# mehta-lab/dynamorph

Measured on AMD Instinct MI355X. Metric: cell-patches/sec (128x128x2) VQ-VAE fwd+bwd, higher is better.
Workload: dtype f32; 1 GPU; C3: VQ_VAE training step (forward + backward + fused Adam), 2x128x128 fp32 synthetic patches; per_gpu_batch=2048, global_batch=2048, parallelism=dp1, hip_graph=True, fused_trainer=True, backward_products=f32

## Files before the change

### dynamorph_amd/csrc/conv_mfma.hip

```cpp
#include "dm_common.h"
#include "tile.h"
#include "mfma_util.h"

int dm_generic_conv_slabs(int B, int per_tile);
int dm_generic_conv(int form, const Operand &in, const WeightView &wv, float *out, const Epilogue &ep, int B, int Cphys,
                    int CIN, int NOUT, int H, int W, int taps, int nslabs, int per_tile, hipStream_t st);
bool dm_wide_conv_ok(int form, int H, int W);
int dm_wide_conv_slabs(int form, int B, int H, int W, int per_tile);
long long dm_wide_conv_scratch_floats(int form, int CIN, int NOUT, int taps);
int dm_wide_conv(int form, const Operand &in, const WeightView &wv, float *scratch, float *out, const Epilogue &ep, int B,
                 int Cphys, int CIN, int NOUT, int H, int W, int taps, int nslabs, int per_tile, hipStream_t st);

bool dm_conv4x4s2_patch_forward(const Operand &in, const WeightView &wv, float *out, const Epilogue &ep, int B, int Cphys, int CIN,
                                int NOUT, int H, int W, int per_tile, int nslabs, hipStream_t stream, int *rc);

namespace {

enum { SIDE_NONE = 0, SIDE_MASK = 1, SIDE_ALL = 2 };

template <int SIDE> struct EpiIn { f32x4 m; };
template <> struct EpiIn<SIDE_ALL> { f32x4 m, r, q; };

constexpr unsigned DM_RSRC_FLAGS = 0x00020000u;
constexpr int DM_VOFF_NONE = 0x40000000;

__device__ __forceinline__ __amdgpu_buffer_rsrc_t sample_rsrc(const float *base, long long sample_elems, int b)
{
    return base ? __builtin_amdgcn_make_buffer_rsrc(const_cast<float *>(base + sample_elems * b), 0,
                                                    (int)(sample_elems * 4), DM_RSRC_FLAGS)
                : __builtin_amdgcn_make_buffer_rsrc(nullptr, 0, 0, DM_RSRC_FLAGS);
}

template <int SIDE> struct EpiCtx {
    __amdgpu_buffer_rsrc_t out_r, m_r, r_r, q_r;
    __device__ __forceinline__ void rebase(const Epilogue &ep, float *out, long long sample_elems, int b)
    {
        out_r = sample_rsrc(out, sample_elems, b);
        if constexpr (SIDE != SIDE_NONE) m_r = sample_rsrc(ep.mask.p0, sample_elems, b);
        if constexpr (SIDE == SIDE_ALL) {
            r_r = sample_rsrc(ep.resid, sample_elems, b);
            q_r = sample_rsrc(ep.stat_q, sample_elems, b);
        }
    }
};

template <int SIDE>
__device__ __forceinline__ void epilogue_loads(EpiIn<SIDE> &e, const EpiCtx<SIDE> &cx, int voff)
{
    if constexpr (SIDE != SIDE_NONE) e.m = __builtin_amdgcn_raw_buffer_load_b128(cx.m_r, voff, 0, 0);
    if constexpr (SIDE == SIDE_ALL) {
        e.r = __builtin_amdgcn_raw_buffer_load_b128(cx.r_r, voff, 0, 0);
        e.q = __builtin_amdgcn_raw_buffer_load_b128(cx.q_r, voff, 0, 0);
    }
}

__device__ __forceinline__ void mask_coef(const Epilogue &ep, int b, int chan, float &c0, float &c2)
{
    c0 = ep.mask.p0 ? 1.f : 0.f; c2 = ep.mask.p0 ? 0.f : 1.f;
    if (ep.mask.p0 && ep.mask.mode >= DM_LOAD_AFFINE) {
        const float *cf = ep.mask.coef + (long long)b * ep.mask.coef_bstride + chan * 4;
        c0 = cf[0]; c2 = cf[2];
    }
}

template <int SIDE>
__device__ __forceinline__ void epilogue_tail(f32x4 v, const Epilogue &ep, const EpiCtx<SIDE> &cx, const EpiIn<SIDE> &e,
                                              float mc0, float mc2, int voff, double &s1, double &s2)
{
    f32x4 q = v;
    if constexpr (SIDE != SIDE_NONE) {
        const f32x4 mv = mc0 * e.m + mc2;
        v.x = mv.x > 0.f ? v.x : 0.f; v.y = mv.y > 0.f ? v.y : 0.f;
        v.z = mv.z > 0.f ? v.z : 0.f; v.w = mv.w > 0.f ? v.w : 0.f;
    }
    if constexpr (SIDE == SIDE_ALL) v += e.r;
    __builtin_amdgcn_raw_buffer_store_b128(v, cx.out_r, voff, 0, 0);
    if (ep.stats) {
        q = v;
        if constexpr (SIDE == SIDE_MASK) { if (ep.stat_q) q = e.m; }
        if constexpr (SIDE == SIDE_ALL) { if (ep.stat_q) q = e.q; }
        s1 += (double)((v.x + v.y) + (v.z + v.w));
        s2 += (double)((v.x * q.x + v.y * q.y) + (v.z * q.z + v.w * q.w));
    }
}

__device__ __forceinline__ f32x4 bias_relu(f32x4 v, const Epilogue &ep, float bias)
{
    v += bias;
    if (ep.relu) v = dm_relu4(v);
    return v;
}

template <int NTT, bool PIX>
__device__ __forceinline__ void stats_reduce(double (&s1)[NTT], double (&s2)[NTT], double (*s_stat)[2],
                                             const Epilogue &ep, int NCH, long long slab)
{
    const int lane = threadIdx.x & 63, wave = threadIdx.x >> 6;
#pragma unroll
    for (int t = 0; t < NTT; ++t) {
        double a = dm_row_sum_f64(s1[t]), c = dm_row_sum_f64(s2[t]);
        if (PIX) {
            a += __shfl_xor(a, 1, 64); c += __shfl_xor(c, 1, 64);
            a += __shfl_xor(a, 2, 64); c += __shfl_xor(c, 2, 64);
        }
        if (lane < 16) {
            s_stat[(wave * NTT + t) * 16 + lane][0] = a;
            s_stat[(wave * NTT + t) * 16 + lane][1] = c;
        }
    }
    __syncthreads();
    for (int ch = threadIdx.x; ch < NCH; ch += DM_BLOCK) {
        const int n = PIX ? ch * 4 : ch;
        const int t = n >> 4, l = n & 15;
        double a = 0.0, c = 0.0;
#pragma unroll
        for (int w = 0; w < 4; ++w) {
            a += s_stat[(w * NTT + t) * 16 + l][0];
            c += s_stat[(w * NTT + t) * 16 + l][1];
        }
        ep.stats[(slab * NCH + ch) * 2 + 0] = a;
        ep.stats[(slab * NCH + ch) * 2 + 1] = c;
    }
}

__device__ __forceinline__ void zero_unowned_slabs(const Epilogue &ep, int NCH, int nslabs)
{
    for (int t2 = blockIdx.x + gridDim.x; t2 < nslabs; t2 += gridDim.x)
        for (int i = threadIdx.x; i < NCH * 2; i += DM_BLOCK) ep.stats[(long long)t2 * NCH * 2 + i] = 0.0;
}

template <int CIN, int NT, int TH, int TW, int SIDE, int WPS, bool BB>
__global__ __launch_bounds__(DM_BLOCK, WPS)
void conv4x4s2_kernel(Operand in, WeightView wv, float *__restrict__ out, Epilogue ep, int Cphys, int NOUT, int H,
                      int W, int ntiles, int nslabs, int per_tile)
{
    constexpr int IH = 2 * TH + 2, RS = 2 * TW + 8, COLS4 = RS / 4, PS = IH * RS;
    constexpr int KS = CIN * 4, CG = TW / 16, MT = TH * CG, MTW = MT / 4;
    constexpr int MP = NT == 1 ? 2 : 1;
    static_assert(MTW % MP == 0 && MTW >= MP, "M tiles per wave");
    __shared__ __attribute__((aligned(16))) float tile[CIN * PS];
    __shared__ __attribute__((aligned(16))) float s_coef[DM_COEF_MAX_C * 4];
    __shared__ double s_stat[4 * NT * 16][2];

    const int Ho = H >> 1, Wo = W >> 1;
    const int tiles_x = Wo / TW, tiles_y = Ho / TH;
    const int lane = threadIdx.x & 63, wave = threadIdx.x >> 6, m = lane & 15, kq = lane >> 4;

    TileStage<CIN, IH, COLS4, RS, PS, false> stage;
    stage.init(H, W);
    int tidx = blockIdx.x, b = 0, oy0 = 0, ox0 = 0;
    if (tidx < ntiles) {
        int t = tidx;
        ox0 = (t % tiles_x) * TW; t /= tiles_x;
        oy0 = (t % tiles_y) * TH; b = t / tiles_y;
        stage.issue(in, b, Cphys, H, W, 2 * oy0 - 1, 2 * ox0 - 4);
        stage_coef(s_coef, in, b, Cphys);
    }

    static_assert(!BB || NT == 1, "bias_border: one N tile");
    float tb00 = 0.f, tb01 = 0.f, tb02 = 0.f, tb10 = 0.f, tb11 = 0.f, tb12 = 0.f, tb20 = 0.f, tb21 = 0.f, tb22 = 0.f;
    if constexpr (BB) {
        const float *tp = ep.bias_border + (m < NOUT ? m : 0);
        tb00 = tp[0 * NOUT]; tb01 = tp[1 * NOUT]; tb02 = tp[2 * NOUT];
        tb10 = tp[3 * NOUT]; tb11 = tp[4 * NOUT]; tb12 = tp[5 * NOUT];
        tb20 = tp[6 * NOUT]; tb21 = tp[7 * NOUT]; tb22 = tp[8 * NOUT];
    }
    float wreg[NT][KS], bias[NT], mc0[NT], mc2[NT];
#pragma unroll
    for (int t = 0; t < NT; ++t) {
        const int n = 16 * t + m;
        const int nc = n < NOUT ? n : 0;
        bias[t] = ep.bias ? ep.bias[nc] : 0.f;
        mask_coef(ep, 0, nc, mc0[t], mc2[t]);
#pragma unroll
        for (int s = 0; s < KS; ++s)
            wreg[t][s] = n < NOUT ? wv.w[wv.off + n * wv.sn + (s >> 2) * wv.sc + (s & 3) * wv.sky + kq * wv.skx] : 0.f;
    }

    double s1[NT], s2[NT];
#pragma unroll
    for (int t = 0; t < NT; ++t) { s1[t] = 0.0; s2[t] = 0.0; }
    const int abase = 2 * m + kq + 3;
    auto off = [](int s) { return (s >> 2) * PS + (s & 3) * RS; };
    EpiCtx<SIDE> cx;
    const long long sample_elems = (long long)NOUT * Ho * Wo;
    int chan_off[NT];
#pragma unroll
    for (int t = 0; t < NT; ++t) chan_off[t] = 16 * t + m < NOUT ? ((16 * t + m) * Ho * Wo + 4 * kq) * 4 : DM_VOFF_NONE;
    while (tidx < ntiles) {
        __syncthreads();
        stage.commit(tile, s_coef, Cphys, H, W, 2 * oy0 - 1, 2 * ox0 - 4, in.mode);
        __syncthreads();
        const int cb = b, cy0 = oy0, cx0 = ox0;
        const int next = tidx + gridDim.x;
        {
            int t = next < ntiles ? next : tidx;
            ox0 = (t % tiles_x) * TW; t /= tiles_x;
            oy0 = (t % tiles_y) * TH; b = t / tiles_y;
        }
        const auto scx = stage.begin(in, next < ntiles, b, Cphys, H, W, 2 * oy0 - 1, 2 * ox0 - 4);
        const bool recoef = next < ntiles && coef_changes(in, cb, b);
        f32x4 cfn = {1.f, 0.f, 0.f, 0.f};
        if (recoef) cfn = coef_fetch(in, b, Cphys);
        if (SIDE != SIDE_NONE && ep.mask.p0 && ep.mask.coef_bstride) {
#pragma unroll
            for (int t = 0; t < NT; ++t) mask_coef(ep, cb, 16 * t + m < NOUT ? 16 * t + m : 0, mc0[t], mc2[t]);
        }
        cx.rebase(ep, out, sample_elems, cb);
        constexpr int NP = MTW / MP, NE = decltype(stage)::N;
#pragma unroll
        for (int p = 0; p < NP; ++p) {
#pragma unroll
            for (int e = 0; e < NE; ++e)
                if (e >= p * NE / NP && e < (p + 1) * NE / NP) stage.issue_one(e, scx);
            const float *ap[MP];
            int o[MP][NT];
            EpiIn<SIDE> e[MP][NT];
#pragma unroll
            for (int i = 0; i < MP; ++i) {
                const int ti = wave + 4 * (MP * p + i);
                const int r = ti / CG, cg = ti % CG;
                ap[i] = tile + (2 * r) * RS + 32 * cg + abase;
#pragma unroll
                for (int t = 0; t < NT; ++t) {
                    o[i][t] = chan_off[t] + ((cy0 + r) * Wo + cx0 + 16 * cg) * 4;
                    epilogue_loads<SIDE>(e[i][t], cx, o[i][t]);
                }
            }
            f32x4 acc[MP][NT];
#pragma unroll
            for (int i = 0; i < MP; ++i)
#pragma unroll
                for (int t = 0; t < NT; ++t) acc[i][t] = (f32x4){0.f, 0.f, 0.f, 0.f};
            mfma_tiles<MP, NT, KS, 4>(ap, wreg, acc, off);
#pragma unroll
            for (int i = 0; i < MP; ++i)
#pragma unroll
                for (int t = 0; t < NT; ++t)
                {
                    f32x4 v = acc[i][t];
                    if constexpr (BB) {
                        const int ti = wave + 4 * (MP * p + i);
                        const int y = cy0 + ti / CG, xq = cx0 + 16 * (ti % CG) + 4 * kq;
                        const bool r0 = y == 0, r2 = y == Ho - 1;
                        const float bl = r0 ? tb00 : (r2 ? tb20 : tb10);
                        const float bm = r0 ? tb01 : (r2 ? tb21 : tb11);
                        const float br = r0 ? tb02 : (r2 ? tb22 : tb12);
                        v += (f32x4){xq == 0 ? bl : bm, bm, bm, xq + 3 == Wo - 1 ? br : bm};
                        v = bias_relu(v, ep, 0.f);
                    } else {
                        v = bias_relu(v, ep, bias[t]);
                    }
                    epilogue_tail<SIDE>(v, ep, cx, e[i][t], mc0[t], mc2[t], o[i][t], s1[t], s2[t]);
                }
        }
        if (per_tile && ep.stats) {
            stats_reduce<NT, false>(s1, s2, s_stat, ep, NOUT, tidx);
#pragma unroll
            for (int t = 0; t < NT; ++t) { s1[t] = 0.0; s2[t] = 0.0; }
        }
        if (recoef) coef_put(s_coef, in, cfn, Cphys);
        tidx = next;
    }
    if (ep.stats && !per_tile) {
        stats_reduce<NT, false>(s1, s2, s_stat, ep, NOUT, blockIdx.x);
        zero_unowned_slabs(ep, NOUT, nslabs);
    }
}

template <int CIN, int TH, int WPS>
__global__ __launch_bounds__(DM_BLOCK, WPS)
void conv4x4s2_pair_kernel(Operand in, WeightView wv, float *__restrict__ out, Epilogue ep, int Cphys, int H, int W, int ntiles,
                           int nslabs, int per_tile)
{
    constexpr int NOUT = 8, TW = 64;
    constexpr int IH = 2 * TH + 2, RS = 2 * TW + 8, COLS4 = RS / 4, PS = IH * RS;
    constexpr int KS = CIN * 2, RPW = TH / 4;
    static_assert(TH % 4 == 0, "rows over four waves");
    __shared__ __attribute__((aligned(16))) float tile[CIN * PS + 64];
    __shared__ __attribute__((aligned(16))) float s_coef[DM_COEF_MAX_C * 4];
    __shared__ double s_stat[4 * 16][2];

    const int Ho = H >> 1, Wo = W >> 1;
    const int tiles_x = Wo / TW, tiles_y = Ho / TH;
    const int lane = threadIdx.x & 63, wave = threadIdx.x >> 6, m = lane & 15, kq = lane >> 4;
    const int co = m & 7, mj = m >> 3;
    const int kyl = kq >> 1, col = kq & 1;

    TileStage<CIN, IH, COLS4, RS, PS, false> stage;
    stage.init(H, W);
    int tidx = blockIdx.x, b = 0, oy0 = 0, ox0 = 0;
    if (tidx < ntiles) {
        int t = tidx;
        ox0 = (t % tiles_x) * TW; t /= tiles_x;
        oy0 = (t % tiles_y) * TH; b = t / tiles_y;
        stage.issue(in, b, Cphys, H, W, 2 * oy0 - 1, 2 * ox0 - 4);
        stage_coef(s_coef, in, b, Cphys);
    }
    if (threadIdx.x < 64) tile[CIN * PS + threadIdx.x] = 0.f;

    const float *tp = ep.bias_border + co;
    const float tb00 = tp[0 * NOUT], tb01 = tp[1 * NOUT], tb02 = tp[2 * NOUT];
    const float tb10 = tp[3 * NOUT], tb11 = tp[4 * NOUT], tb12 = tp[5 * NOUT];
    const float tb20 = tp[6 * NOUT], tb21 = tp[7 * NOUT], tb22 = tp[8 * NOUT];
    float wc[1][KS], ws[1][KS];
#pragma unroll
    for (int s = 0; s < KS; ++s) {
        const int c = s >> 1, ky = 2 * (s & 1) + kyl;
        const long long base = wv.off + co * wv.sn + c * wv.sc + ky * wv.sky;
        wc[0][s] = wv.w[base + (col + (mj ? 0 : 2)) * wv.skx];
        ws[0][s] = wv.w[base + (col + (mj ? 2 : 0)) * wv.skx];
    }
    float mc0, mc2;
    mask_coef(ep, 0, co, mc0, mc2);
// ... 615 lines not shown
                        }
                    } else {
#pragma unroll
                        for (int i = 0; i < MP; ++i) v[i] = acc[i][0];
                    }
#pragma unroll
                    for (int i = 0; i < MP; ++i) {
                        const f32x4 pv = lane_xor8(v[i]);
                        epilogue_tail<SIDE_MASK>(pxl ? (f32x4){pv.z, v[i].z, pv.w, v[i].w} : (f32x4){v[i].x, pv.x, v[i].y, pv.y}, ep, cx,
                                                 e[i], mc0, mc2, obase[i] + py * OW * 4, s1, s2);
                    }
                }
            }
            }
            __syncthreads();
            p ^= 1;
            tidx += gridDim.x;
        }
        for (int w = 0; w < RW + 1; ++w) __syncthreads();
        if (ep.stats) {
            double a = s1, c = s2;
            a += __shfl_xor(a, 16, 64); c += __shfl_xor(c, 16, 64);
            a += __shfl_xor(a, 32, 64); c += __shfl_xor(c, 32, 64);
            a += __shfl_xor(a, 8, 64); c += __shfl_xor(c, 8, 64);
            if (lane < CX) { s_stat[rw * 16 + lane][0] = a; s_stat[rw * 16 + lane][1] = c; }
        }
        __syncthreads();
        if (ep.stats && threadIdx.x < CX) {
            double ta = 0.0, tc = 0.0;
#pragma unroll
            for (int w = 0; w < RW; ++w) { ta += s_stat[w * 16 + threadIdx.x][0]; tc += s_stat[w * 16 + threadIdx.x][1]; }
            ep.stats[((long long)blockIdx.x * CX + threadIdx.x) * 2 + 0] = ta;
            ep.stats[((long long)blockIdx.x * CX + threadIdx.x) * 2 + 1] = tc;
        }
    }
    float *slab = wslabs + (long long)blockIdx.x * (CD * N);
    for (int i = threadIdx.x; i < NTT * 256; i += 768) {
        const int j = i & 3, l = (i >> 2) & 63, t = i >> 8;
        slab[(4 * (l >> 4) + j) * N + 16 * t + (l & 15)] = fb_lds[i];
    }
}

struct ConvArgs {
    Operand in; WeightView wv; float *out; Epilogue ep;
    int B, Cphys, CIN, NOUT, H, W, per_tile;
    hipStream_t stream;
};

int side_mode(const Epilogue &ep)
{
    if (!ep.mask.p0 && !ep.resid && !ep.stat_q) return SIDE_NONE;
    if (ep.mask.p0 && !ep.resid && (!ep.stat_q || ep.stat_q == ep.mask.p0)) return SIDE_MASK;
    return SIDE_ALL;
}

int conv_grid(int ntiles, int wgs_per_cu, int per_tile, int npass = 1)
{
    if (per_tile && npass > 1) return ntiles;
    const int cap = 256 * wgs_per_cu;
    return ntiles < cap ? ntiles : cap;
}

int conv_slabs(int ntiles, int per_tile) { return per_tile ? ntiles : (ntiles < 256 * 3 ? ntiles : 256 * 3); }

constexpr int lds_wgs(int lds_bytes) { return (160 * 1024) / (lds_bytes + 3072); }
constexpr int clampi(int v, int lo, int hi) { return v < lo ? lo : (v > hi ? hi : v); }

constexpr int conv_wps(int lds_bytes, int weights, int tile_f4, bool two, int mp, int nt, int side)
{
    const int stage = ((tile_f4 + DM_BLOCK - 1) / DM_BLOCK) * (two ? 9 : 5);
    const int epi = mp * nt * (6 + (side == SIDE_ALL ? 12 : (side == SIDE_MASK ? 4 : 0)));
    const int est = weights + stage + epi + 48;
    return clampi(lds_wgs(lds_bytes), 1, est > 145 ? 2 : 3);
}

int conv4_tw(int CIN, int Wo)
{
    const int cap = CIN <= 5 ? 64 : (CIN <= 8 ? 32 : 16);
    return Wo < cap ? Wo : cap;
}

template <int CIN, int TW>
void launch_conv4(const ConvArgs &a)
{
    constexpr int TH = 8;
    constexpr int F4 = CIN * (2 * TH + 2) * ((2 * TW + 8) / 4), LDS = 16 * F4;
    const int ntiles = a.B * ((a.H / 2) / TH) * ((a.W / 2) / TW);
#define DM_L4(SIDE_)                                                                                              \
    {                                                                                                             \
        constexpr int WPS = conv_wps(LDS, CIN * 4, F4, false, 2, 1, SIDE_);                                       \
                                           \
        if (SIDE_ == SIDE_NONE && CIN <= 4 && TW == 64 && a.NOUT == 8 && a.ep.bias_border && !a.ep.relu)             \
            hipLaunchKernelGGL((conv4x4s2_pair_kernel<CIN <= 4 ? CIN : 1, TH, WPS>),                                   \
                               dim3(conv_grid(ntiles, WPS, a.per_tile)), dim3(DM_BLOCK), 0, a.stream, a.in, a.wv,     \
                               a.out, a.ep, a.Cphys, a.H, a.W, ntiles, conv_slabs(ntiles, a.per_tile), a.per_tile);    \
        else if (SIDE_ == SIDE_NONE && CIN <= 5 && a.ep.bias_border)                                              \
            hipLaunchKernelGGL((conv4x4s2_kernel<CIN, 1, TH, TW, SIDE_NONE, WPS, true>),                              \
                               dim3(conv_grid(ntiles, WPS, a.per_tile)), dim3(DM_BLOCK), 0, a.stream, a.in, a.wv,     \
                               a.out, a.ep, a.Cphys, a.NOUT, a.H, a.W, ntiles, conv_slabs(ntiles, a.per_tile),        \
                               a.per_tile);                                                                           \
        else                                                                                                      \
            hipLaunchKernelGGL((conv4x4s2_kernel<CIN, 1, TH, TW, SIDE_, WPS, false>),                                 \
                               dim3(conv_grid(ntiles, WPS, a.per_tile)), dim3(DM_BLOCK), 0, a.stream, a.in, a.wv,     \
                               a.out, a.ep, a.Cphys, a.NOUT, a.H, a.W, ntiles, conv_slabs(ntiles, a.per_tile),        \
                               a.per_tile);                                                                           \
    }
    switch (side_mode(a.ep)) {
    case SIDE_NONE: DM_L4(SIDE_NONE) break;
    case SIDE_MASK: DM_L4(SIDE_MASK) break;
    default: DM_L4(SIDE_ALL)
    }
#undef DM_L4
}

int conv3_tw(int W, int CIN)
{
    const int cap = CIN >= 32 ? 16 : (CIN >= 16 ? 32 : 64);
    return W < cap ? W : cap;
}
constexpr int conv3_th(int TW, int CIN) { return (TW == 16 && CIN < 32) ? 16 : 8; }

template <int CIN, int NT, int NPASS, int TAPS, bool PIX, int TW>
void launch_conv3(const ConvArgs &a)
{
    constexpr int TH = conv3_th(TW, CIN);
    constexpr int PADR = TAPS == 9 ? 1 : 0;
    constexpr int F4 = CIN * (TH + 2 * PADR) * ((TW + 8 * PADR) / 4), LDS = 16 * F4 + 2048;
    const int ntiles = a.B * (a.H / TH) * (a.W / TW);
    const int side = side_mode(a.ep);
    const bool two = a.in.mode == DM_LOAD_AFFINE2;
#define DM_L3(TWO_, SIDE_)                                                                                        \
    {                                                                                                             \
        constexpr int WPS = conv_wps(LDS, NT * (CIN / 4) * TAPS, F4, TWO_, NT == 1 ? 2 : 1, NT, SIDE_);          \
        hipLaunchKernelGGL((conv3x3_kernel<CIN, NT, NPASS, TAPS, PIX, TH, TW, TWO_, SIDE_, WPS>),                 \
                           dim3(conv_grid(ntiles, WPS, a.per_tile, NPASS)), dim3(DM_BLOCK), 0, a.stream, a.in, a.wv, \
                           a.out, a.ep, a.Cphys, a.NOUT, a.H, a.W, ntiles, conv_slabs(ntiles, a.per_tile), a.per_tile); \
    }
    if (!two && side == SIDE_NONE) DM_L3(false, SIDE_NONE)
    else if (!two && side == SIDE_MASK) DM_L3(false, SIDE_MASK)
    else if (two && side != SIDE_ALL) DM_L3(true, SIDE_MASK)
    else DM_L3(true, SIDE_ALL)
#undef DM_L3
}

template <int CIN, int COUT, int TW>
void launch_convT_phase(const ConvArgs &a)
{
    constexpr int TH = conv3_th(TW, CIN);
    constexpr int F4 = CIN * (TH + 2) * ((TW + 8) / 4), LDS = 16 * F4 + 2048;
    constexpr int KSW = (CIN / 4) * (COUT == 16 ? 4 : 6) * (COUT == 16 ? 4 : 2);
    const int ntiles = a.B * (a.H / TH) * (a.W / TW);
    const int side = side_mode(a.ep);
    const bool two = a.in.mode == DM_LOAD_AFFINE2;
#define DM_LP(TWO_, SIDE_)                                                                                        \
    {                                                                                                             \
        constexpr int WPS = clampi(conv_wps(LDS, KSW, F4, TWO_, 2, COUT == 16 ? 2 : 1, SIDE_), 1, 2);             \
        hipLaunchKernelGGL((convT_phase_kernel<CIN, COUT, TH, TW, TWO_, SIDE_, WPS>),                             \
                           dim3(conv_grid(ntiles, WPS, a.per_tile)), dim3(DM_BLOCK), 0, a.stream, a.in, a.wv,     \
                           a.out, a.ep, a.Cphys, a.H, a.W, ntiles, conv_slabs(ntiles, a.per_tile));               \
    }
    if (!two && side == SIDE_NONE) DM_LP(false, SIDE_NONE)
    else if (!two && side == SIDE_MASK) DM_LP(false, SIDE_MASK)
    else if (two && side != SIDE_ALL) DM_LP(true, SIDE_MASK)
    else DM_LP(true, SIDE_ALL)
#undef DM_LP
}

}

static int conv_common_checks(const char *who, const dm_operand *in, const dm_weight_view *w, float *out,
                              const dm_epilogue *ep, int B, int CIN, int NOUT, int H, int W)
{
    if (dm_check_operand(in, who)) return -1;
    DM_REQUIRE(w && w->w && out, "%s: NULL weight or output", who);
    DM_REQUIRE(B > 0 && CIN > 0 && NOUT > 0 && H > 0 && W > 0, "%s: bad shape", who);
    DM_REQUIRE((long long)B * (CIN > NOUT ? CIN : NOUT) * H * W < (1LL << 31),
               "%s: tensor too large for 32-bit element offsets", who);
    DM_REQUIRE(CIN - (in->ones_channel ? 1 : 0) > 0, "%s: no physical input channel", who);
    DM_REQUIRE((long long)NOUT * H * W * 4 < DM_VOFF_NONE, "%s: one output sample must stay below 1 GiB", who);
    if (ep && ep->mask.p0 && dm_check_operand(&ep->mask, who)) return -1;
    DM_REQUIRE(!(ep && ep->mask.p0 && ep->mask.ones_channel), "%s: mask operand cannot have a ones channel", who);
    DM_REQUIRE(!(ep && ep->mask.p0 && ep->mask.mode != DM_LOAD_IDENT && ep->mask.mode != DM_LOAD_AFFINE),
               "%s: mask operand must be IDENT or AFFINE", who);
    return 0;
}

static int conv4_fast_tw(int CIN, int NOUT, int H, int W)
{
    const int Wo = W / 2, Ho = H / 2;
    const int TW = conv4_tw(CIN, Wo);
    if (H % 16 || W % 32 || NOUT > 16 || (TW != 16 && TW != 32 && TW != 64) || Ho % 8 || Wo % TW) return 0;
    return TW;
}

static bool conv4_has_kernel(int CIN, int TW)
{
    if (CIN >= 1 && CIN <= 5) return TW == 64 || TW == 32 || TW == 16;
    if (CIN == 8) return TW == 32 || TW == 16;
    return CIN == 16 && TW == 16;
}

extern "C" int dm_conv4x4s2_num_blocks(int B, int CIN, int NOUT, int H, int W, int per_tile)
{
    if (B <= 0 || H <= 0 || W <= 0 || (H & 1) || (W & 1)) return -1;
    const int TW = conv4_fast_tw(CIN, NOUT, H, W);
    if (TW && conv4_has_kernel(CIN, TW)) return conv_slabs(B * ((H / 2) / 8) * ((W / 2) / TW), per_tile);
    if (dm_wide_conv_ok(0, H, W)) return dm_wide_conv_slabs(0, B, H, W, per_tile);
    return dm_generic_conv_slabs(B, per_tile);
}

extern "C" int64_t dm_conv4x4s2_scratch_floats(int CIN, int NOUT, int H, int W, int fallback)
{
    if (CIN <= 0 || NOUT <= 0 || !dm_wide_conv_ok(0, H, W)) return 0;
    const int TW = conv4_fast_tw(CIN, NOUT, H, W);
    if (TW && conv4_has_kernel(CIN, TW) && !fallback) return 0;
    return dm_wide_conv_scratch_floats(0, CIN, NOUT, 16);
}

extern "C" int dm_conv4x4s2(const dm_operand *in, const dm_weight_view *w, float *out, const dm_epilogue *ep,
                            int B, int CIN, int NOUT, int H, int W, void *stream)
{
    if (conv_common_checks("dm_conv4x4s2", in, w, out, ep, B, CIN, NOUT, H, W)) return -1;
    DM_REQUIRE(H % 2 == 0 && W % 2 == 0, "dm_conv4x4s2: H and W must be even (got %dx%d)", H, W);
    ConvArgs a{to_dev(in), to_dev(w), out, to_dev(ep), B, CIN - (in->ones_channel ? 1 : 0), CIN, NOUT, H, W,
               ep ? ep->stats_per_tile : 0, (hipStream_t)stream};
    {
        int rc = 0;
        if (dm_conv4x4s2_patch_forward(a.in, a.wv, out, a.ep, B, a.Cphys, CIN, NOUT, H, W, a.per_tile,
                                       dm_conv4x4s2_num_blocks(B, CIN, NOUT, H, W, a.per_tile), a.stream, &rc))
            return rc;
    }
    const int TW = conv4_fast_tw(CIN, NOUT, H, W);
    const bool border_ok = !(ep && ep->bias_border) || (CIN <= 5 && !ep->mask.p0 && !ep->resid && !ep->stat_q && W / 2 >= 8);
    if (TW && conv4_has_kernel(CIN, TW) && in->mode != DM_LOAD_AFFINE2 && border_ok) {
#define DM_C4(C, T) if (CIN == C && TW == T) { launch_conv4<C, T>(a); return dm_launch_status("dm_conv4x4s2"); }
        DM_C4(3, 64) DM_C4(3, 32) DM_C4(3, 16)
        DM_C4(4, 64) DM_C4(4, 32) DM_C4(4, 16)
        DM_C4(5, 64) DM_C4(5, 32) DM_C4(5, 16)
        DM_C4(2, 64) DM_C4(2, 32) DM_C4(2, 16)
        DM_C4(1, 64) DM_C4(1, 32) DM_C4(1, 16)
        DM_C4(8, 32) DM_C4(8, 16)
        DM_C4(16, 16)
#undef DM_C4
    }
    const int nslabs = dm_conv4x4s2_num_blocks(B, CIN, NOUT, H, W, a.per_tile);
    if (dm_wide_conv_ok(0, H, W) && w->scratch && w->scratch_floats >= dm_wide_conv_scratch_floats(0, CIN, NOUT, 16))
        dm_wide_conv(0, a.in, a.wv, w->scratch, out, a.ep, B, a.Cphys, CIN, NOUT, H, W, 16, nslabs, a.per_tile, a.stream);
    else
        dm_generic_conv(0, a.in, a.wv, out, a.ep, B, a.Cphys, CIN, NOUT, H, W, 16, nslabs, a.per_tile, a.stream);
    return dm_launch_status("dm_conv4x4s2");
}

static bool conv3_fast_tileable(int CIN, int H, int W)
{
    const int TW = conv3_tw(W, CIN), TH = conv3_th(TW, CIN);
    return (TW == 16 || TW == 32 || TW == 64) && W % TW == 0 && H % TH == 0 && CIN % 4 == 0 && CIN <= 32;
}

static bool conv3_has_kernel(int CIN, int NOUT, int H, int W, int taps, bool pix, int per_tile)
{
    if (!conv3_fast_tileable(CIN, H, W)) return false;
    const int TW = conv3_tw(W, CIN), NTT = (NOUT + 15) / 16;
    const bool t13 = TW == 16 || TW == 32;
    if (pix && CIN == 16 && (NOUT == 32 || NOUT == 64) && t13 && !per_tile) return true;
    if (!pix && taps == 9) return t13 && ((CIN == 16 && (NTT == 1 || NTT == 2)) || (CIN == 32 && NTT == 1));
    if (!pix && taps == 1) return t13 && ((CIN == 32 && NTT == 1) || (CIN == 16 && NTT == 2));
    if (pix && taps == 9) {
        if (CIN == 16 && NTT == 2) return true;
        if (CIN == 16 && NTT == 4) return t13;
        if (CIN == 8 && NTT == 1) return TW == 32 || TW == 64;
        if (CIN == 4 && NTT == 1) return TW == 64;
    }
    return false;
}

extern "C" int dm_conv3x3_num_blocks(int B, int CIN, int NOUT, int H, int W, int taps, int pixel_shuffle, int per_tile)
{
    if (B <= 0 || H <= 0 || W <= 0) return -1;
    if (conv3_has_kernel(CIN, NOUT, H, W, taps, pixel_shuffle != 0, per_tile)) {
        const int TW = conv3_tw(W, CIN), TH = conv3_th(TW, CIN);
        return conv_slabs(B * (H / TH) * (W / TW), per_tile);
    }
    const int form = pixel_shuffle ? 2 : 1;
    if (dm_wide_conv_ok(form, H, W)) return dm_wide_conv_slabs(form, B, H, W, per_tile);
    return dm_generic_conv_slabs(B, per_tile);
}

extern "C" int64_t dm_conv3x3_scratch_floats(int CIN, int NOUT, int H, int W, int taps, int pixel_shuffle, int per_tile)
{
    const int form = pixel_shuffle ? 2 : 1;
    if (CIN <= 0 || NOUT <= 0 || (taps != 9 && taps != 1) || !dm_wide_conv_ok(form, H, W)) return 0;
    if (conv3_has_kernel(CIN, NOUT, H, W, taps, pixel_shuffle != 0, per_tile)) return 0;
    return dm_wide_conv_scratch_floats(form, CIN, NOUT, taps);
}

extern "C" int dm_conv3x3(const dm_operand *in, const dm_weight_view *w, float *out, const dm_epilogue *ep,
                          int B, int CIN, int NOUT, int H, int W, int taps, int pixel_shuffle, void *stream)
{
    if (conv_common_checks("dm_conv3x3", in, w, out, ep, B, CIN, NOUT, H, W)) return -1;
    DM_REQUIRE(taps == 9 || taps == 1, "dm_conv3x3: taps must be 9 or 1");
    DM_REQUIRE(!pixel_shuffle || (taps == 9 && NOUT % 4 == 0), "dm_conv3x3: pixel_shuffle needs taps=9, NOUT%%4==0");
    DM_REQUIRE(!in->ones_channel, "dm_conv3x3: ones_channel not supported");
    DM_REQUIRE(!(ep && ep->bias_border), "dm_conv3x3: bias_border not supported (dm_conv4x4s2 only)");
    const int TW = conv3_tw(W, CIN);
    const bool fast = conv3_has_kernel(CIN, NOUT, H, W, taps, pixel_shuffle != 0, ep ? ep->stats_per_tile : 0);
    ConvArgs a{to_dev(in), to_dev(w), out, to_dev(ep), B, CIN, CIN, NOUT, H, W, ep ? ep->stats_per_tile : 0,
               (hipStream_t)stream};
    const int NTT = (NOUT + 15) / 16;
    const bool pix = pixel_shuffle != 0;
    if (fast) {
#define DM_CP(CO, T)                                                                       \
    if (pix && CIN == 16 && NOUT == 4 * CO && TW == T && !a.per_tile) {                    \
        launch_convT_phase<16, CO, T>(a);                                                  \
        return dm_launch_status("dm_conv3x3");                                             \
    }
    DM_CP(8, 16) DM_CP(8, 32) DM_CP(16, 16) DM_CP(16, 32)
#undef DM_CP
#define DM_C3(C, NTOT, NT_, NP_, TP, PX, T)                                                \
    if (CIN == C && NTT == NTOT && taps == TP && pix == PX && TW == T) {                   \
        launch_conv3<C, NT_, NP_, TP, PX, T>(a);                                           \
        return dm_launch_status("dm_conv3x3");                                             \
    }
    DM_C3(16, 1, 1, 1, 9, false, 16) DM_C3(16, 1, 1, 1, 9, false, 32)
    DM_C3(16, 2, 2, 1, 9, false, 16) DM_C3(16, 2, 2, 1, 9, false, 32)
    DM_C3(32, 1, 1, 1, 9, false, 16) DM_C3(32, 1, 1, 1, 9, false, 32)
    DM_C3(32, 1, 1, 1, 1, false, 16) DM_C3(32, 1, 1, 1, 1, false, 32)
    DM_C3(16, 2, 2, 1, 1, false, 16) DM_C3(16, 2, 2, 1, 1, false, 32)
    DM_C3(16, 2, 2, 1, 9, true, 16) DM_C3(16, 2, 2, 1, 9, true, 32) DM_C3(16, 2, 2, 1, 9, true, 64)
    DM_C3(16, 4, 2, 2, 9, true, 16) DM_C3(16, 4, 2, 2, 9, true, 32)
    DM_C3(8, 1, 1, 1, 9, true, 32) DM_C3(8, 1, 1, 1, 9, true, 64)
    DM_C3(4, 1, 1, 1, 9, true, 64)
#undef DM_C3
    }
    const int nslabs = dm_conv3x3_num_blocks(B, CIN, NOUT, H, W, taps, pixel_shuffle, a.per_tile);
    if (fast) {
        dm_set_error("dm_conv3x3: kernel table and conv3_has_kernel disagree (CIN %d NOUT %d %dx%d)", CIN, NOUT, H, W);
        return -1;
    }
    if (dm_wide_conv_ok(pix ? 2 : 1, H, W) && w->scratch &&
        w->scratch_floats >= dm_wide_conv_scratch_floats(pix ? 2 : 1, CIN, NOUT, taps))
        dm_wide_conv(pix ? 2 : 1, a.in, a.wv, w->scratch, out, a.ep, B, CIN, CIN, NOUT, H, W, taps, nslabs, a.per_tile, a.stream);
    else
        dm_generic_conv(pix ? 2 : 1, a.in, a.wv, out, a.ep, B, CIN, CIN, NOUT, H, W, taps, nslabs, a.per_tile, a.stream);
    return dm_launch_status("dm_conv3x3");
}


static bool fused_bwd_shape(int CD, int CX, int H, int W)
{
    return CD == 16 && CX == 8 && H > 0 && W > 0 && H % 8 == 0 && W % 32 == 0;
}

extern "C" int dm_conv_bwd_s2_fused_supported(int CD, int CX, int H, int W) { return fused_bwd_shape(CD, CX, H, W) ? 1 : 0; }

extern "C" int dm_backward_precision(int mode)
{
    DM_REQUIRE(mode != 1, "dm_backward_precision: the split-bf16 gradient kernels are not built (retired: slower than the "
                          "exact fp32 path on these layer widths)");
    return 0;
}

extern "C" int dm_conv_bwd_s2_fused_num_blocks(int B, int CD, int CX, int H, int W)
{
    if (B <= 0 || !fused_bwd_shape(CD, CX, H, W)) return -1;
    const long long ntiles = (long long)B * (H / 8) * (W / 32);
    const long long cap = 256;
    return (int)(ntiles < cap ? ntiles : cap);
}

extern "C" int dm_conv_bwd_s2_fused(const dm_operand *dy, const dm_operand *tin, const dm_weight_view *w, float *dx,
                                    const dm_epilogue *ep, float *w_slabs, int B, int CD, int CX, int H, int W,
                                    void *stream)
{
    if (dm_check_operand(dy, "dm_conv_bwd_s2_fused(dy)") || dm_check_operand(tin, "dm_conv_bwd_s2_fused(in)")) return -1;
    DM_REQUIRE(w && w->w && dx && w_slabs && ep, "dm_conv_bwd_s2_fused: NULL pointer");
    DM_REQUIRE(fused_bwd_shape(CD, CX, H, W), "dm_conv_bwd_s2_fused: shape %d -> %d channels on %dx%d not built", CX, CD, H, W);
    DM_REQUIRE(B > 0 && (long long)B * CD * 4 * H * W < (1LL << 31), "dm_conv_bwd_s2_fused: tensor too large for 32-bit offsets");
    DM_REQUIRE(!dy->ones_channel && !tin->ones_channel && tin->mode != DM_LOAD_AFFINE2,
               "dm_conv_bwd_s2_fused: operand modes");
    DM_REQUIRE(dy->coef_bstride == 0 && tin->coef_bstride == 0, "dm_conv_bwd_s2_fused: batch-statistics coefficients only");
    DM_REQUIRE(ep->mask.p0 == tin->p0 && (!ep->stat_q || ep->stat_q == tin->p0) && !ep->resid && !ep->bias && !ep->relu &&
                   ep->mask.coef_bstride == 0,
               "dm_conv_bwd_s2_fused: the epilogue must mask by (and take its statistics against) the layer input");
    if (dm_check_operand(&ep->mask, "dm_conv_bwd_s2_fused(mask)")) return -1;
    using G = FusedBwdGeom<16, 8, 8, 32>;
    using G64 = FusedBwdGeom<16, 8, 4, 64>;
    static DmPerDeviceOnce attr_set;
    if (attr_set.need()) {
        hipError_t e = hipFuncSetAttribute((const void *)bwd_s2_roles3_kernel<16, 8, 8, 32, false>,
                                           hipFuncAttributeMaxDynamicSharedMemorySize, (int)G::LDS_BYTES);
        if (e == hipSuccess)
            e = hipFuncSetAttribute((const void *)bwd_s2_roles3_kernel<16, 8, 8, 32, true>,
                                    hipFuncAttributeMaxDynamicSharedMemorySize, (int)G::LDS_BYTES);
        if (e == hipSuccess)
            e = hipFuncSetAttribute((const void *)bwd_s2_roles3_kernel<16, 8, 4, 64, true>,
                                    hipFuncAttributeMaxDynamicSharedMemorySize, (int)G64::LDS_BYTES);
        if (e != hipSuccess) { dm_set_error("dm_conv_bwd_s2_fused: cannot reserve %zu bytes of LDS: %s", G::LDS_BYTES, hipGetErrorString(e)); return (int)e; }
        attr_set.mark();
    }
    const int ntiles = B * (H / 8) * (W / 32);
    const int grid = dm_conv_bwd_s2_fused_num_blocks(B, CD, CX, H, W);
    if (W == 64 && H % 4 == 0)
        hipLaunchKernelGGL((bwd_s2_roles3_kernel<16, 8, 4, 64, true>), dim3(grid), dim3(768), G64::LDS_BYTES, (hipStream_t)stream,
                           to_dev(dy), to_dev(tin), to_dev(w), dx, to_dev(ep), w_slabs, H, W, B * (H / 4), 0);
    else if (W == 32)
        hipLaunchKernelGGL((bwd_s2_roles3_kernel<16, 8, 8, 32, true>), dim3(grid), dim3(768), G::LDS_BYTES, (hipStream_t)stream,
                           to_dev(dy), to_dev(tin), to_dev(w), dx, to_dev(ep), w_slabs, H, W, ntiles, 0);
    else
        hipLaunchKernelGGL((bwd_s2_roles3_kernel<16, 8, 8, 32, false>), dim3(grid), dim3(768), G::LDS_BYTES, (hipStream_t)stream,
                           to_dev(dy), to_dev(tin), to_dev(w), dx, to_dev(ep), w_slabs, H, W, ntiles, 0);
    return dm_launch_status("dm_conv_bwd_s2_fused");
}
```

Before: 1.042 million patches/s.

## Add Winograd F(2x2,3x3) MFMA kernel for 16-channel 16x16 conv3x3

Adds a Winograd F(2,3) 3x3 convolution kernel for CIN=16, NOUT=16/32 on 16x16 images and routes matching dm_conv3x3 calls to it ahead of the existing direct MFMA kernels. Weights are transformed in double precision per block, input tiles are transformed in registers from LDS, and the 16 per-tile elementwise products run as MFMA 16x16x4 ops before the output transform and the fused epilogue (bias, relu, mask, residual, stats). The aim is to cut multiply work on these small layers, at the cost of Winograd rounding differences, per-block weight-transform overhead, and a fixed grid of up to 768 blocks.

```diff
diff --git a/dynamorph_amd/csrc/conv3x3_wino.hip b/dynamorph_amd/csrc/conv3x3_wino.hip
--- /dev/null
+++ b/dynamorph_amd/csrc/conv3x3_wino.hip
@@ -0,0 +1,263 @@
+#include "dm_common.h"
+
+namespace {
+
+constexpr int WN_CIN = 16, WN_HW = 16, WN_ROWS = 6, WN_RS = 24, WN_PS = 160, WN_WAVES = 4;
+
+enum { WN_SIDE_NONE = 0, WN_SIDE_MASK = 1, WN_SIDE_ALL = 2 };
+
+int wn_side_mode(const Epilogue &ep)
+{
+    if (!ep.mask.p0 && !ep.resid && !ep.stat_q) return WN_SIDE_NONE;
+    if (ep.mask.p0 && !ep.resid && (!ep.stat_q || ep.stat_q == ep.mask.p0)) return WN_SIDE_MASK;
+    return WN_SIDE_ALL;
+}
+
+template <int SIDE>
+__device__ __forceinline__ void wn_epilogue(f32x4 v, const Epilogue &ep, float *__restrict__ outb, long long sb, int o, float mc0,
+                                            float mc2, double &s1, double &s2)
+{
+    f32x4 q = v;
+    if constexpr (SIDE != WN_SIDE_NONE) {
+        f32x4 mr = {0.f, 0.f, 0.f, 0.f};
+        if (ep.mask.p0) mr = *reinterpret_cast<const f32x4 *>(ep.mask.p0 + sb + o);
+        const f32x4 mv = mc0 * mr + mc2;
+        v.x = mv.x > 0.f ? v.x : 0.f; v.y = mv.y > 0.f ? v.y : 0.f;
+        v.z = mv.z > 0.f ? v.z : 0.f; v.w = mv.w > 0.f ? v.w : 0.f;
+        if constexpr (SIDE == WN_SIDE_ALL) { if (ep.resid) v += *reinterpret_cast<const f32x4 *>(ep.resid + sb + o); }
+        q = v;
+        if constexpr (SIDE == WN_SIDE_MASK) { if (ep.stat_q) q = mr; }
+    }
+    if constexpr (SIDE == WN_SIDE_ALL) { if (ep.stat_q) q = *reinterpret_cast<const f32x4 *>(ep.stat_q + sb + o); }
+    *reinterpret_cast<f32x4 *>(outb + o) = v;
+    if (ep.stats) {
+        s1 += (double)((v.x + v.y) + (v.z + v.w));
+        s2 += (double)((v.x * q.x + v.y * q.y) + (v.z * q.z + v.w * q.w));
+    }
+}
+
+template <int NT, bool TWO, int SIDE>
+__global__ __launch_bounds__(64 * WN_WAVES, NT == 1 ? 2 : 1)
+void conv3x3_wino_kernel(Operand in, WeightView wv, float *__restrict__ out, Epilogue ep, int B)
+{
+    constexpr int NOUT = 16 * NT, PS = WN_PS, RS = WN_RS;
+    __shared__ __attribute__((aligned(16))) float wn_lds[WN_WAVES * WN_CIN * WN_PS];
+    __shared__ double s_stat[WN_WAVES][NOUT][2];
+    __shared__ __attribute__((aligned(16))) float s_u[4 * NT * 4 * 64 * 4];
+
+    const int lane = threadIdx.x & 63, m = lane & 15, kq = lane >> 4;
+    const int wave = __builtin_amdgcn_readfirstlane(threadIdx.x >> 6);
+    float *img = wn_lds + wave * WN_CIN * PS;
+
+    for (int i = lane; i < WN_CIN * PS / 4; i += 64) reinterpret_cast<f32x4 *>(img)[i] = (f32x4){0.f, 0.f, 0.f, 0.f};
+
+    {
+        const int ks = wave;
+#pragma unroll
+        for (int t = 0; t < NT; ++t) {
+            const float *wp = wv.w + wv.off + (16 * t + m) * wv.sn + (4 * ks + kq) * wv.sc;
+            double g[3][3], h[4][3];
+#pragma unroll
+            for (int ky = 0; ky < 3; ++ky)
+#pragma unroll
+                for (int kx = 0; kx < 3; ++kx) g[ky][kx] = (double)wp[ky * wv.sky + kx * wv.skx];
+#pragma unroll
+            for (int j = 0; j < 3; ++j) {
+                h[0][j] = g[0][j];
+                h[1][j] = 0.5 * (g[0][j] + g[1][j] + g[2][j]);
+                h[2][j] = 0.5 * (g[0][j] - g[1][j] + g[2][j]);
+                h[3][j] = g[2][j];
+            }
+#pragma unroll
+            for (int a = 0; a < 4; ++a)
+                *reinterpret_cast<f32x4 *>(s_u + (((ks * NT + t) * 4 + a) * 64 + lane) * 4) =
+                    (f32x4){(float)h[a][0], (float)(0.5 * (h[a][0] + h[a][1] + h[a][2])),
+                            (float)(0.5 * (h[a][0] - h[a][1] + h[a][2])), (float)h[a][2]};
+        }
+    }
+    __syncthreads();
+    float bias[NT];
+#pragma unroll
+    for (int t = 0; t < NT; ++t) bias[t] = ep.bias ? ep.bias[16 * t + m] : 0.f;
+    double s1[NT], s2[NT];
+#pragma unroll
+    for (int t = 0; t < NT; ++t) { s1[t] = 0.0; s2[t] = 0.0; }
+
+    constexpr long long IN_SAMPLE = WN_CIN * WN_HW * WN_HW, OUT_SAMPLE = NOUT * WN_HW * WN_HW;
+    const int sc = lane >> 2, sx = 4 * (lane & 3);
+    const int sl = sc * PS + sx + 1, sg = sc * WN_HW * WN_HW + (4 * wave - 1) * WN_HW + sx;
+    auto row_ok = [&](int j) { return (unsigned)(4 * wave - 1 + j) < (unsigned)WN_HW; };
+    int b = blockIdx.x;
+    f32x4 rv[WN_ROWS];
+    auto fetch = [&](const float *p, int bb, f32x4 (&r)[WN_ROWS]) {
+#pragma unroll
+        for (int j = 0; j < WN_ROWS; ++j)
+            r[j] = row_ok(j) ? *reinterpret_cast<const f32x4 *>(p + bb * IN_SAMPLE + sg + j * WN_HW) : (f32x4){0.f, 0.f, 0.f, 0.f};
+    };
+    if (b < B) fetch(in.p0, b, rv);
+    const int wbase = kq * PS + 2 * (m >> 3) * RS + 2 * (m & 7);
+    const int obase = (4 * wave + 2 * (kq >> 1)) * WN_HW + 8 * (kq & 1);
+
+    for (; b < B; b += gridDim.x) {
+        float c0 = 1.f, c1 = 0.f, c2 = 0.f;
+        if (in.mode >= DM_LOAD_AFFINE) {
+            const float *cf = in.coef + (long long)b * in.coef_bstride + sc * 4;
+            c0 = cf[0]; c1 = cf[1]; c2 = cf[2];
+        }
+        f32x4 ru[WN_ROWS];
+        if (TWO) fetch(in.p1, b, ru);
+#pragma unroll
+        for (int j = 0; j < WN_ROWS; ++j) {
+            f32x4 v = rv[j];
+            if (TWO) {
+                v = c0 * v + c2;
+                v += c1 * ru[j];
+            } else if (in.mode == DM_LOAD_RELU) {
+                v = dm_relu4(v);
+            } else if (in.mode >= DM_LOAD_AFFINE) {
+                v = c0 * v + c2;
+                if (in.mode == DM_LOAD_AFFINE_RELU) v = dm_relu4(v);
+            }
+            if (!row_ok(j)) v = (f32x4){0.f, 0.f, 0.f, 0.f};
+            float *d = img + sl + j * RS;
+            d[0] = v.x;
+            *reinterpret_cast<f32x2 *>(d + 1) = (f32x2){v.y, v.z};
+            d[3] = v.w;
+        }
+        if (b + (int)gridDim.x < B) fetch(in.p0, b + gridDim.x, rv);
+        float mc0[NT], mc2[NT];
+#pragma unroll
+        for (int t = 0; t < NT; ++t) {
+            mc0[t] = ep.mask.p0 ? 1.f : 0.f; mc2[t] = ep.mask.p0 ? 0.f : 1.f;
+            if (SIDE != WN_SIDE_NONE && ep.mask.p0 && ep.mask.mode >= DM_LOAD_AFFINE) {
+                const float *mcf = ep.mask.coef + (long long)b * ep.mask.coef_bstride + (16 * t + m) * 4;
+                mc0[t] = mcf[0]; mc2[t] = mcf[2];
+            }
+        }
+        const long long sb = b * OUT_SAMPLE;
+        float *outb = out + sb;
+
+        float v[4][16];
+        const float *wp = img + wbase;
+#pragma unroll
+        for (int ks = 0; ks < 4; ++ks) {
+            float d[4][4];
+#pragma unroll
+            for (int r = 0; r < 4; ++r) {
+                const f32x2 lo = *reinterpret_cast<const f32x2 *>(wp + 4 * ks * PS + r * RS);
+                const f32x2 hi = *reinterpret_cast<const f32x2 *>(wp + 4 * ks * PS + r * RS + 2);
+                d[r][0] = lo.x; d[r][1] = lo.y; d[r][2] = hi.x; d[r][3] = hi.y;
+            }
+            float e[4][4];
+#pragma unroll
+            for (int j = 0; j < 4; ++j) {
+                e[0][j] = d[0][j] - d[2][j];
+                e[1][j] = d[1][j] + d[2][j];
+                e[2][j] = d[2][j] - d[1][j];
+                e[3][j] = d[1][j] - d[3][j];
+            }
+#pragma unroll
+            for (int i = 0; i < 4; ++i) {
+                v[ks][4 * i + 0] = e[i][0] - e[i][2];
+                v[ks][4 * i + 1] = e[i][1] + e[i][2];
+                v[ks][4 * i + 2] = e[i][2] - e[i][1];
+                v[ks][4 * i + 3] = e[i][1] - e[i][3];
+            }
+        }
+#pragma unroll
+        for (int t = 0; t < NT; ++t) {
+            f32x4 acc[16];
+#pragma unroll
+            for (int p = 0; p < 16; ++p) acc[p] = (f32x4){0.f, 0.f, 0.f, 0.f};
+#pragma unroll
+            for (int ks = 0; ks < 4; ++ks)
+#pragma unroll
+                for (int a = 0; a < 4; ++a) {
+                    const f32x4 ub = *reinterpret_cast<const f32x4 *>(s_u + (((ks * NT + t) * 4 + a) * 64 + lane) * 4);
+                    acc[4 * a + 0] = __builtin_amdgcn_mfma_f32_16x16x4f32(v[ks][4 * a + 0], ub.x, acc[4 * a + 0], 0, 0, 0);
+                    acc[4 * a + 1] = __builtin_amdgcn_mfma_f32_16x16x4f32(v[ks][4 * a + 1], ub.y, acc[4 * a + 1], 0, 0, 0);
+                    acc[4 * a + 2] = __builtin_amdgcn_mfma_f32_16x16x4f32(v[ks][4 * a + 2], ub.z, acc[4 * a + 2], 0, 0, 0);
+                    acc[4 * a + 3] = __builtin_amdgcn_mfma_f32_16x16x4f32(v[ks][4 * a + 3], ub.w, acc[4 * a + 3], 0, 0, 0);
+                }
+            float y[4][4];
+#pragma unroll
+            for (int r = 0; r < 4; ++r) {
+                float o0[4], o1[4];
+#pragma unroll
+                for (int j = 0; j < 4; ++j) {
+                    o0[j] = acc[j][r] + acc[4 + j][r] + acc[8 + j][r];
+                    o1[j] = acc[4 + j][r] - acc[8 + j][r] - acc[12 + j][r];
+                }
+                y[r][0] = o0[0] + o0[1] + o0[2];
+                y[r][1] = o0[1] - o0[2] - o0[3];
+                y[r][2] = o1[0] + o1[1] + o1[2];
+                y[r][3] = o1[1] - o1[2] - o1[3];
+            }
+            const int o = (16 * t + m) * WN_HW * WN_HW + obase;
+            f32x4 q[4] = {(f32x4){y[0][0], y[0][1], y[1][0], y[1][1]}, (f32x4){y[2][0], y[2][1], y[3][0], y[3][1]},
+                          (f32x4){y[0][2], y[0][3], y[1][2], y[1][3]}, (f32x4){y[2][2], y[2][3], y[3][2], y[3][3]}};
+#pragma unroll
+            for (int k = 0; k < 4; ++k) {
+                f32x4 vv = q[k] + bias[t];
+                if (ep.relu) vv = dm_relu4(vv);
+                wn_epilogue<SIDE>(vv, ep, outb, sb, o + (k >> 1) * WN_HW + 4 * (k & 1), mc0[t], mc2[t], s1[t], s2[t]);
+            }
+        }
+    }
+
+    if (ep.stats) {
+#pragma unroll
+        for (int t = 0; t < NT; ++t) {
+            const double a = dm_row_sum_f64(s1[t]), c = dm_row_sum_f64(s2[t]);
+            if (lane < 16) { s_stat[wave][16 * t + lane][0] = a; s_stat[wave][16 * t + lane][1] = c; }
+        }
+        __syncthreads();
+        if ((int)threadIdx.x < 2 * NOUT) {
+            const int ch = threadIdx.x >> 1, k = threadIdx.x & 1;
+            double a = 0.0;
+#pragma unroll
+            for (int w = 0; w < WN_WAVES; ++w) a += s_stat[w][ch][k];
+            ep.stats[((long long)blockIdx.x * NOUT + ch) * 2 + k] = a;
+        }
+    }
+}
+
+template <int NT, bool TWO, int SIDE>
+hipError_t wn_launch(const Operand &in, const WeightView &wv, float *out, const Epilogue &ep, int B, int grid, hipStream_t st)
+{
+    hipLaunchKernelGGL((conv3x3_wino_kernel<NT, TWO, SIDE>), dim3(grid), dim3(64 * WN_WAVES), 0, st, in, wv, out, ep, B);
+    return hipGetLastError();
+}
+
+template <int NT>
+hipError_t wn_dispatch(const Operand &in, const WeightView &wv, float *out, const Epilogue &ep, int B, int grid, hipStream_t st)
+{
+    const int side = wn_side_mode(ep);
+    const bool two = in.mode == DM_LOAD_AFFINE2;
+    if (!two && side == WN_SIDE_NONE) return wn_launch<NT, false, WN_SIDE_NONE>(in, wv, out, ep, B, grid, st);
+    if (!two && side == WN_SIDE_MASK) return wn_launch<NT, false, WN_SIDE_MASK>(in, wv, out, ep, B, grid, st);
+    if (!two) return wn_launch<NT, false, WN_SIDE_ALL>(in, wv, out, ep, B, grid, st);
+    if (side != WN_SIDE_ALL) return wn_launch<NT, true, WN_SIDE_MASK>(in, wv, out, ep, B, grid, st);
+    return wn_launch<NT, true, WN_SIDE_ALL>(in, wv, out, ep, B, grid, st);
+}
+
+}
+
+bool dm_conv3x3_wino_route(int CIN, int NOUT, int H, int W, int taps, int pixel_shuffle, int per_tile)
+{
+    return CIN == WN_CIN && (NOUT == 16 || NOUT == 32) && H == WN_HW && W == WN_HW && taps == 9 && !pixel_shuffle && !per_tile;
+}
+
+int dm_conv3x3_wino_slabs(int B) { return B < 768 ? B : 768; }
+
+int dm_conv3x3_wino(const Operand &in, const WeightView &wv, float *out, const Epilogue &ep, int B, int NOUT, hipStream_t st)
+{
+    DM_REQUIRE((long long)B * 32 * WN_HW * WN_HW < (1LL << 31), "dm_conv3x3: tensor too large for 32-bit offsets");
+    const int grid = dm_conv3x3_wino_slabs(B);
+    const hipError_t e = NOUT == 32 ? wn_dispatch<2>(in, wv, out, ep, B, grid, st) : wn_dispatch<1>(in, wv, out, ep, B, grid, st);
+    if (e != hipSuccess) {
+        dm_set_error("dm_conv3x3 (Winograd): %s", hipGetErrorString(e));
+        return -1;
+    }
+    return 0;
+}
diff --git a/dynamorph_amd/csrc/conv_mfma.hip b/dynamorph_amd/csrc/conv_mfma.hip
--- a/dynamorph_amd/csrc/conv_mfma.hip
+++ b/dynamorph_amd/csrc/conv_mfma.hip
@@ -10,6 +10,9 @@
 long long dm_wide_conv_scratch_floats(int form, int CIN, int NOUT, int taps);
 int dm_wide_conv(int form, const Operand &in, const WeightView &wv, float *scratch, float *out, const Epilogue &ep, int B,
                  int Cphys, int CIN, int NOUT, int H, int W, int taps, int nslabs, int per_tile, hipStream_t st);
+
+bool dm_conv3x3_wino_route(int CIN, int NOUT, int H, int W, int taps, int pixel_shuffle, int per_tile);
+int dm_conv3x3_wino(const Operand &in, const WeightView &wv, float *out, const Epilogue &ep, int B, int NOUT, hipStream_t st);
 
 bool dm_conv4x4s2_patch_forward(const Operand &in, const WeightView &wv, float *out, const Epilogue &ep, int B, int Cphys, int CIN,
                                 int NOUT, int H, int W, int per_tile, int nslabs, hipStream_t stream, int *rc);
@@ -1231,6 +1234,8 @@
     DM_REQUIRE(!pixel_shuffle || (taps == 9 && NOUT % 4 == 0), "dm_conv3x3: pixel_shuffle needs taps=9, NOUT%%4==0");
     DM_REQUIRE(!in->ones_channel, "dm_conv3x3: ones_channel not supported");
     DM_REQUIRE(!(ep && ep->bias_border), "dm_conv3x3: bias_border not supported (dm_conv4x4s2 only)");
+    if (dm_conv3x3_wino_route(CIN, NOUT, H, W, taps, pixel_shuffle, ep ? ep->stats_per_tile : 0))
+        return dm_conv3x3_wino(to_dev(in), to_dev(w), out, to_dev(ep), B, NOUT, (hipStream_t)stream);
     const int TW = conv3_tw(W, CIN);
     const bool fast = conv3_has_kernel(CIN, NOUT, H, W, taps, pixel_shuffle != 0, ep ? ep->stats_per_tile : 0);
     ConvArgs a{to_dev(in), to_dev(w), out, to_dev(ep), B, CIN, CIN, NOUT, H, W, ep ? ep->stats_per_tile : 0,
```

New measurement: 1.053 million patches/s (median of 6 runs). About the same (+1.0%).
